# HybridRobotics/ilqr-iterative-tasks

Hardware: AMD Instinct MI355X
Metric: batched iLQR iterations/s (n=6,m=2,N=20) (higher is better)
Workload: dtype f64

## Files before the change

### ilqr_iterative_tasks_amd/csrc/i2lqr_group.hip

```cpp
#include "i2lqr_group.h"

#include "i2lqr_devcfg.hpp"
#include "i2lqr_geometry.hpp"
#include "i2lqr_group.hpp"
#include "i2lqr_dryrun.hpp"

namespace i2lqr {

namespace {

template <class T, class Sys, int G = kGroup> size_t group_lds_bytes(int N) {
  return (size_t)GLayout<Sys, G>(N).wave_words() * sizeof(T);
}

bool has_stage_weights(const i2lqr_config& cfg) {
  for (int i = 0; i < cfg.n; i++)
    for (int j = 0; j < cfg.n; j++)
      if (cfg.Q[i * I2LQR_MAX_N + j] != 0.0) return true;
  for (int a = 0; a < cfg.m; a++)
    for (int b = 0; b < cfg.m; b++)
      if (cfg.R[a * I2LQR_MAX_M + b] != 0.0) return true;
  return false;
}

template <auto Kernel> hipError_t raise_lds_limit(size_t lds) {
  if (lds <= device_geometry().default_dyn_lds) return hipSuccess;
  constexpr int kMaxDev = 64;
  static thread_local int raised_for[kMaxDev] = {};
  int dev = 0;
  hipError_t e = hipGetDevice(&dev);
  if (e != hipSuccess) return e;
  if (dev < 0 || dev >= kMaxDev || raised_for[dev] < (int)lds) {
    e = hipFuncSetAttribute((const void*)Kernel, hipFuncAttributeMaxDynamicSharedMemorySize,
                            (int)lds);
    if (e != hipSuccess) return e;
    if (dev >= 0 && dev < kMaxDev) raised_for[dev] = (int)lds;
  }
  return hipSuccess;
}

template <class T, class Sys, int H, int G = kGroup>
hipError_t launch_h(const i2lqr_config& cfg, const IterArgs<T>& a, hipStream_t s) {
  const auto c = make_dev_cfg<T, Sys::n, Sys::m>(cfg);
  const size_t lds = group_lds_bytes<T, Sys, G>(cfg.N);
  if (hipError_t e = raise_lds_limit<k_group_iterate<T, Sys, H, false, G>>(lds); e != hipSuccess)
    return e;
  constexpr int PW = 64 / G;
  const unsigned grid = (unsigned)((a.B + PW - 1) / PW);
  hipLaunchKernelGGL((k_group_iterate<T, Sys, H, false, G>), dim3(grid), dim3(64 * H), lds, s, c, a,
                     (T*)nullptr);
  return hipGetLastError();
}
template <class T, class Sys>
hipError_t launch16(const i2lqr_config& cfg, const IterArgs<T>& a, hipStream_t s) {
  const int64_t cus = device_geometry().cus;
#ifndef I2LQR_STAMPS
  if ((a.B + 3) / 4 <= 2 * cus) return launch_h<T, Sys, 2, 16>(cfg, a, s);
#endif
  return launch_h<T, Sys, 1, 16>(cfg, a, s);
}
template <class T, class Sys>
hipError_t launch_ws(const i2lqr_config& cfg, const IterArgs<T>& a, void* ws, hipStream_t s) {
  const auto c = make_dev_cfg<T, Sys::n, Sys::m>(cfg);
  const size_t lds = (size_t)GLayout<Sys>(cfg.N, true).wave_words() * sizeof(T);
  if (hipError_t e = raise_lds_limit<k_group_iterate<T, Sys, 1, true>>(lds); e != hipSuccess) return e;
  const unsigned grid = (unsigned)((a.B + kGroupsPerWave - 1) / kGroupsPerWave);
  hipLaunchKernelGGL((k_group_iterate<T, Sys, 1, true>), dim3(grid), dim3(64), lds, s, c, a, (T*)ws);
  return hipGetLastError();
}

template <class T, class Sys>
hipError_t launch(const i2lqr_config& cfg, const IterArgs<T>& a, hipStream_t s) {
  const int64_t cus = device_geometry().cus;
#ifndef I2LQR_STAMPS
  if ((a.B + kGroupsPerWave - 1) / kGroupsPerWave <= cus) return launch_h<T, Sys, 3>(cfg, a, s);
#endif
  return launch_h<T, Sys, 1>(cfg, a, s);
}

constexpr int kSpecWideBatch = 512;

template <class T, class Sys, int V, int G = kGroup> size_t spec_lds_bytes(int N) {
  return (size_t)GSpecLayout<Sys, V, G>(N).group_words() * sizeof(T);
}

template <class T, class Sys, int V, bool SETIO, int G>
hipError_t launch_spec_v(const i2lqr_config& cfg, const IterArgs<T>& a, hipStream_t s) {
  const auto c = make_dev_cfg<T, Sys::n, Sys::m>(cfg);
  const size_t lds = spec_lds_bytes<T, Sys, V, G>(cfg.N);
  if (hipError_t e = raise_lds_limit<k_group_spec<T, Sys, V, SETIO, G>>(lds); e != hipSuccess)
    return e;
  constexpr int PW = 64 / G;
  const int64_t problems = SETIO ? (int64_t)a.count_max : a.B;
  const unsigned grid = (unsigned)((problems + PW - 1) / PW);
  hipLaunchKernelGGL((k_group_spec<T, Sys, V, SETIO, G>), dim3(grid), dim3(64 * V), lds, s, c, a);
  return hipGetLastError();
}
template <class T, class Sys, bool SETIO, int G>
hipError_t launch_spec(const i2lqr_config& cfg, const IterArgs<T>& a, hipStream_t s) {
  const DeviceGeometry& geo = device_geometry();
  const bool wide = !SETIO && a.B <= geo.scaled(kSpecWideBatch) &&
                    spec_lds_bytes<T, Sys, 3, G>(cfg.N) <= geo.max_dyn_lds;
  if (wide) return launch_spec_v<T, Sys, 3, SETIO, G>(cfg, a, s);
  return launch_spec_v<T, Sys, 2, SETIO, G>(cfg, a, s);
}
template <class T, bool SETIO>
hipError_t launch_spec_any(const i2lqr_config& cfg, const IterArgs<T>& a, hipStream_t s, int lanes) {
  const bool b4 = cfg.system_id == I2LQR_SYS_BICYCLE4;
  if (lanes == 16)
    return b4 ? launch_spec<T, Bicycle4<T>, SETIO, 16>(cfg, a, s)
              : launch_spec<T, Bicycle6<T>, SETIO, 16>(cfg, a, s);
  return b4 ? launch_spec<T, Bicycle4<T>, SETIO, kGroup>(cfg, a, s)
            : launch_spec<T, Bicycle6<T>, SETIO, kGroup>(cfg, a, s);
}

template <int G> bool spec_lds_fits(const i2lqr_config& cfg) {
  const size_t lds = cfg.dtype == I2LQR_F64
      ? (cfg.system_id == I2LQR_SYS_BICYCLE4 ? spec_lds_bytes<double, Bicycle4<double>, 2, G>(cfg.N)
                                             : spec_lds_bytes<double, Bicycle6<double>, 2, G>(cfg.N))
      : (cfg.system_id == I2LQR_SYS_BICYCLE4 ? spec_lds_bytes<float, Bicycle4<float>, 2, G>(cfg.N)
                                             : spec_lds_bytes<float, Bicycle6<float>, 2, G>(cfg.N));
  return lds <= device_geometry().max_dyn_lds;
}
bool spec_plant_ok(const i2lqr_config& cfg) {
  if (cfg.system_id != I2LQR_SYS_BICYCLE4 && cfg.system_id != I2LQR_SYS_BICYCLE6) return false;
  return !has_stage_weights(cfg);
}

}

bool group_spec_supported(const i2lqr_config& cfg, int lanes) {
  if (!spec_plant_ok(cfg) || cfg.layout != I2LQR_LAYOUT_PROBLEM_MAJOR) return false;
  return lanes == 16 ? spec_lds_fits<16>(cfg) : (group_supported(cfg) && spec_lds_fits<kGroup>(cfg));
}
int group_spec_tail_lanes(const i2lqr_config& cfg) {
  if (!spec_plant_ok(cfg)) return 0;
  return spec_lds_fits<16>(cfg) ? 16 : (spec_lds_fits<kGroup>(cfg) ? kGroup : 0);
}
bool group_spec_tail_supported(const i2lqr_config& cfg) { return group_spec_tail_lanes(cfg) != 0; }

template <class T, class Sys>
hipError_t launch_spec_chain(const i2lqr_config& cfg, const IterArgs<T>& a, hipStream_t s) {
  const auto c = make_dev_cfg<T, Sys::n, Sys::m>(cfg);
  const size_t lds = spec_lds_bytes<T, Sys, 3, 16>(cfg.N);
  if (hipError_t e = raise_lds_limit<k_group_spec<T, Sys, 3, false, 16, true>>(lds); e != hipSuccess)
    return e;
  const unsigned grid = (unsigned)((a.B + 3) / 4);
  hipLaunchKernelGGL((k_group_spec<T, Sys, 3, false, 16, true>), dim3(grid), dim3(64 * 3), lds, s, c, a);
  return hipGetLastError();
}
bool group_spec_chain_supported(const i2lqr_config& cfg, int64_t chains) {
  if (!spec_plant_ok(cfg) || cfg.layout != I2LQR_LAYOUT_PROBLEM_MAJOR) return false;
  const DeviceGeometry& geo = device_geometry();
  if (chains > geo.scaled(kSpecWideBatch)) return false;
  const size_t lds = cfg.dtype == I2LQR_F64
      ? (cfg.system_id == I2LQR_SYS_BICYCLE4 ? spec_lds_bytes<double, Bicycle4<double>, 3, 16>(cfg.N)
                                             : spec_lds_bytes<double, Bicycle6<double>, 3, 16>(cfg.N))
      : (cfg.system_id == I2LQR_SYS_BICYCLE4 ? spec_lds_bytes<float, Bicycle4<float>, 3, 16>(cfg.N)
// ... 103 lines not shown
```

### ilqr_iterative_tasks_amd/csrc/i2lqr_group.hpp

```cpp
#pragma once
#include <hip/hip_runtime.h>
#include <stdint.h>

#include "i2lqr_systems.hpp"
#include "i2lqr_wave.hpp"

namespace i2lqr {

constexpr int kGroup = 8;
constexpr int kGroupsPerWave = 64 / kGroup;

template <class Sys> struct GroupPattern {
  static constexpr int n = Sys::n, m = Sys::m, W = n + m, NV = Sys::NVAR;
  static constexpr int dt_row(int b) {
    for (int i = 2; i < n; i++)
      if (i != b && Sys::pat(i, b) == 2) return i;
    return -1;
  }
  static constexpr bool column_ok(int b) {
    int extra = 0;
    for (int i = 0; i < n; i++) {
      const int code = Sys::pat(i, b);
      if (i < 2) {
        if (code == 2) return false;
        if (i == b && code != 1) return false;
        continue;
      }
      if (i == b) {
        if (code != 1) return false;
      } else if (code == 2) {
        extra++;
      } else if (code != 0) {
        return false;
      }
    }
    return extra <= 1;
  }
  static constexpr bool ok() {
    if (W > kGroup || n + 1 > kGroup || n < 2) return false;
    for (int b = 0; b < W; b++)
      if (!column_ok(b)) return false;
    return true;
  }
};

#ifndef I2LQR_GROUP_UNROLL
#define I2LQR_GROUP_UNROLL 4
#endif
template <class Sys, int G = kGroup> struct GLayout {
  static constexpr int n = Sys::n, m = Sys::m, W = n + m, NV = Sys::NVAR, NT = Sys::NTRIG;
  static constexpr int PW = 64 / G;
  static constexpr int KW = (n + 1 + 1) & ~1;
  static constexpr int R_JV = 0, R_ZERO = NV, R_ONE = NV + 1, R_LU = NV + 2, R_LUU = NV + 2 + m,
                       R_OB = NV + 2 + 2 * m, RW = (NV + 2 + 2 * m + 5 + 1) & ~1;
  int N;
  static constexpr int kT1Stride = 80;
  int XU0, XU1, Kk, R, TR0, TR1, total;
  __host__ __device__ explicit GLayout(int N_, bool ws = false) : N(N_) {
    int o = 0;
    XU0 = o; o += W * (N + 1); o = (o + 3) & ~3;
    XU1 = o; o += W * (N + 1); o = (o + 3) & ~3;
    Kk = o; o += ws ? m * KW : m * KW * N; o = (o + 3) & ~3;
    R = o; o += ws ? 0 : RW * (N + 1);
    TR0 = o; o += NT * (N + 1); o = (o + 3) & ~3;
    TR1 = o; o += NT * (N + 1); o = (o + 3) & ~3;
    o = (o + 3) & ~3;
    if (((o / 4) & 1) == 0) o += 4;
    total = o;
  }
  __host__ __device__ int t1_base() const { return PW * total; }
  __host__ __device__ int qt_base() const { return t1_base() + (G == kGroup ? PW * kT1Stride : 0); }
  __host__ __device__ int ctl_base() const { return (qt_base() + n * n + 3) & ~3; }
  __host__ __device__ int wave_words() const { return ctl_base() + 16; }
  __host__ __device__ int ws_rec() const { return 0; }
  __host__ __device__ int ws_gain() const { return RW * (N + 1); }
  __host__ __device__ int ws_words() const { return (RW * (N + 1) + m * KW * N + 15) & ~15; }
};


template <int L> __device__ __forceinline__ void bcast_fmac1(double& a, double s, double c) {
  asm("v_fmac_f64_dpp %0, %1, %2 row_newbcast:%3 row_mask:0xf bank_mask:0xf" : "+v"(a) : "v"(s), "v"(c), "n"(L));
}
template <int L> __device__ __forceinline__ void bcast_fmac1(float& a, float s, float c) {
  asm("v_fmac_f32_dpp %0, %1, %2 row_newbcast:%3 row_mask:0xf bank_mask:0xf" : "+v"(a) : "v"(s), "v"(c), "n"(L));
}
template <int L, class T, int R>
__device__ __forceinline__ void bcast_fmac(T (&a)[R], const T (&s)[R], T c) {
#pragma unroll
  for (int r = 0; r < R; r++) bcast_fmac1<L>(a[r], s[r], c);
}
template <int L> __device__ __forceinline__ double bcast_mov(double v) {
  long long x = __builtin_bit_cast(long long, v);
  x = __builtin_amdgcn_mov_dpp(x, 0x150 + L, 0xf, 0xf, false);
  return __builtin_bit_cast(double, x);
}
template <int L> __device__ __forceinline__ float bcast_mov(float v) {
  int x = __builtin_bit_cast(int, v);
  x = __builtin_amdgcn_mov_dpp(x, 0x150 + L, 0xf, 0xf, false);
  return __builtin_bit_cast(float, x);
}
template <class T, int R> __device__ __forceinline__ void dpp_ready(T (&v)[R]) {
  if constexpr (R == 8)
    asm("s_nop 1" : "+v"(v[0]), "+v"(v[1]), "+v"(v[2]), "+v"(v[3]), "+v"(v[4]), "+v"(v[5]), "+v"(v[6]), "+v"(v[7]));
  else if constexpr (R == 6)
    asm("s_nop 1" : "+v"(v[0]), "+v"(v[1]), "+v"(v[2]), "+v"(v[3]), "+v"(v[4]), "+v"(v[5]));
  else static_assert(R == 6 || R == 8, "dpp_ready: n + m of the bicycles");
}

template <class T, class Sys, bool WS = false, int G = kGroup> struct GroupWorker {
  static constexpr int n = Sys::n, m = Sys::m, W = n + m, NV = Sys::NVAR, NT = Sys::NTRIG;
  static constexpr int NA = n + 1;
  using Cfg = DevCfg<T, n, m>;
  using GL = GLayout<Sys, G>;
  static_assert(G == kGroup || G == 16, "eight lanes per problem, or one 16-lane DPP row");
  static_assert(G == kGroup || !WS, "the workspace form is built for eight lanes per problem");
  using GP = GroupPattern<Sys>;
  static_assert(GP::ok(), "plant does not have the column structure this kernel is written for");
  const Cfg& c;
  const GL L;
  const Slice<T> S;
  const T* const Qt;
  const int g;
  const int N;
  int oR, oKk;
  T* T1c;
  int rho;
  T* Wp = nullptr;

  int off_c0, off_c1;
  int off_l0, off_l1;
  int off_lu[m];
  T own, cdt;
  int rsrc;
#ifdef I2LQR_STAMPS
  mutable unsigned long long st_acc[8] = {0, 0, 0, 0, 0, 0, 0, 0}, st_t0 = 0, st_t1 = 0;
#endif

  __device__ GroupWorker(const Cfg& c_, T* smem, int lane)
      : GroupWorker(c_, smem + (lane / G) * GL(c_.N, WS).total,
                    smem + GL(c_.N, WS).qt_base(), lane % G,
                    GL(c_.N, WS).total) {
    const int p = lane / G;
    if constexpr (G == kGroup) T1c = smem + L.t1_base() + p * GL::kT1Stride;
    rho = (p >> 1) & 1;
  }
  __device__ __forceinline__ T* rec(int t) const {
    if constexpr (WS) return Wp + L.ws_rec() + t * GL::RW;
    else return S + oR + t * GL::RW;
  }
  __device__ __forceinline__ T* gain(int t) const {
    if constexpr (WS) return Wp + L.ws_gain() + t * (m * GL::KW);
    else return S + oKk + t * (m * GL::KW);
  }
  __device__ __forceinline__ T* gain_x(int t) const {
    if constexpr (WS) return S + oKk;
    else return S + oKk + t * (m * GL::KW);
  }
  __device__ __forceinline__ void ws_publish() const {
    if constexpr (WS) {
      __builtin_amdgcn_fence(__ATOMIC_RELEASE, "workgroup");
      __builtin_amdgcn_s_waitcnt(0);
      wave_sync();
      __builtin_amdgcn_fence(__ATOMIC_ACQUIRE, "workgroup");
    }
  }
  __device__ __forceinline__ int t1_word(int col, int row) const {
    return (row >> 1) * (2 * kGroup) + ((col + rho) & (kGroup - 1)) * 2 + (row & 1);
  }

  __device__ GroupWorker(const Cfg& c_, T* slice, const T* qt, int g_, int slice_words)
      : c(c_), L(c_.N, WS), S(make_slice(slice, slice_words, c_.trap, TAG_GROUP_LDS)), Qt(qt),
        g(g_), N(c_.N) {
    oR = L.R; oKk = L.Kk;
    T1c = nullptr;
    rho = 0;
    off_c0 = GL::R_ZERO; off_c1 = GL::R_ZERO; off_l0 = GL::R_ZERO; off_l1 = GL::R_ZERO;
#pragma unroll
    for (int a = 0; a < m; a++) off_lu[a] = GL::R_ZERO;
    own = T(0); cdt = T(0); rsrc = 0;
    static_for_i<0, W>([&](auto b_) {
      constexpr int b = decltype(b_)::value;
      if (g == b && b < n) {
        constexpr int c0 = Sys::pat(0, b), c1 = Sys::pat(1, b);
        off_c0 = c0 == 0 ? GL::R_ZERO : (c0 == 1 ? GL::R_ONE : GL::R_JV + (c0 - 3));
        off_c1 = c1 == 0 ? GL::R_ZERO : (c1 == 1 ? GL::R_ONE : GL::R_JV + (c1 - 3));
        own = (b >= 2) ? T(1) : T(0);
        constexpr int r = GP::dt_row(b);
        cdt = r >= 0 ? c.dt : T(0);
        rsrc = r >= 0 ? r : 0;
        if (b < 2) {
          off_l0 = GL::R_OB + 2 + b;
          off_l1 = GL::R_OB + 3 + b;
        }
      }
    });
    if (g == n) {
      own = T(1);
      off_l0 = GL::R_OB + 0;
      off_l1 = GL::R_OB + 1;
#pragma unroll
      for (int a = 0; a < m; a++) off_lu[a] = GL::R_LU + a;
    }
    if constexpr (G == 16) {
      own = T(1);
      if (g == 0) off_c0 = GL::R_ZERO;
      if (g == 1) off_c1 = GL::R_ZERO;
    }
  }

  __device__ __forceinline__ T terminal_cost(const T (&x)[n], const T (&xT)[n]) const {
    T d[n];
#pragma unroll
    for (int i = 0; i < n; i++) d[i] = x[i] - xT[i];
    T acc = T(0);
#pragma unroll
    for (int j = 0; j < n; j++) {
      T col = T(0);
#pragma unroll
      for (int i = 0; i < n; i++) col += d[i] * Qt[i * n + j];
      acc += col * d[j];
    }
    return acc;
  }

  template <int i, int a> __device__ __forceinline__ void f_acc(T& acc, bool& first, T v,
                                                                const T (&jv)[NV]) const {
    constexpr int code = Sys::pat(i, a);
    if constexpr (code == 0) {
      return;
    } else if constexpr (code == 1) {
      acc = first ? v : acc + v;
      first = false;
    } else {
      const T f = code == 2 ? c.dt : jv[code >= 3 ? code - 3 : 0];
      acc = first ? f * v : t_fma(f, v, acc);
      first = false;
    }
  }

  __device__ __forceinline__ T rollout(int XUo, int TRo, const T (&xT)[n]) const {
    T x[n], u[m], xn[n], tr[NT];
#pragma unroll
    for (int i = 0; i < n; i++) x[i] = S[XUo + i];
    for (int t = 0; t < N; t++) {
#pragma unroll
      for (int a = 0; a < m; a++) u[a] = clip(S[XUo + t * W + n + a], -c.u_max[a], c.u_max[a]);
#pragma unroll
      for (int a = 0; a < m; a++) S[XUo + t * W + n + a] = u[a];
      Sys::trig(x, tr);
#pragma unroll
      for (int q = 0; q < NT; q++) S[TRo + t * NT + q] = tr[q];
      Sys::step_tr(c, x, u, tr, xn);
#pragma unroll
      for (int i = 0; i < n; i++) S[XUo + (t + 1) * W + i] = xn[i];
#pragma unroll
      for (int i = 0; i < n; i++) x[i] = xn[i];
    }
    Sys::trig(x, tr);
#pragma unroll
    for (int q = 0; q < NT; q++) S[TRo + N * NT + q] = tr[q];
    const T cost = terminal_cost(x, xT);
    wave_sync();
    return cost;
  }

  __device__ __forceinline__ void prep(int XUo, int TRo, const T (&ob)[6], T pa, T pb, int first,
                                       int stride) const {
    const bool has_ob = ob[5] >= T(0);
    const int opt = has_ob ? (int)ob[5] : 0;
    const T spd_y = opt == 1 ? ob[4] : T(0), spd_x = opt == 2 ? ob[4] : T(0);
    const int rounds = (N + stride) / stride;
    for (int r = 0; r < rounds; r++) {
      const int t0 = first + r * stride;
      const int t = t0 < N ? t0 : N;
      const int ts = t0 < N ? t0 : N - 1;
      T* Rs = rec(ts);
      {
        T xe[n], tr[NT], u[m], jv[NV];
#pragma unroll
        for (int i = 0; i < n; i++) xe[i] = S[XUo + (ts + 1) * W + i];
#pragma unroll
        for (int a = 0; a < m; a++) u[a] = S[XUo + ts * W + n + a];
#pragma unroll
        for (int q = 0; q < NT; q++) tr[q] = S[TRo + (ts + 1) * NT + q];
        Sys::jac_var(c, xe, u, tr, jv);
#pragma unroll
        for (int q = 0; q < NV; q++) Rs[GL::R_JV + q] = jv[q];
#pragma unroll
        for (int a = 0; a < m; a++) {
          T e_hi, e_lo;
          if (sizeof(T) == 8 && c.fast_barrier) {
            e_hi = t_exp_bounded(c.ctrl_q2 * (u[a] - c.u_max[a]));
            e_lo = c.ctrl_c[a] * t_rcp(e_hi);
          } else {
            e_hi = t_exp(c.ctrl_q2 * (u[a] - c.u_max[a]));
            e_lo = t_exp(c.ctrl_q2 * (-c.u_max[a] - u[a]));
          }
          Rs[GL::R_LU + a] = c.ctrl_q12 * e_hi - c.ctrl_q12 * e_lo;
          Rs[GL::R_LUU + a] = c.ctrl_q122 * e_hi +
                              c.ctrl_q122 * e_lo;
        }
      }
      T* R = rec(t);
      R[GL::R_ZERO] = T(0);
      R[GL::R_ONE] = T(1);
      const T px = S[XUo + t * W + 0], py = S[XUo + t * W + 1];
      const T dz = opt == 2 ? px - (ob[0] - T(t) * spd_x) : px - ob[0];
      const T dy = opt == 1 ? py - (ob[1] + T(t) * spd_y) : py - ob[1];
      const T h = T(1) + c.safety_margin - (dz * pa * dz + dy * pb * dy);
      const T hd0 = T(-2) * pa * dz, hd1 = T(-2) * pb * dy;
      const T e = t_exp(c.obs_q2 * h);
      const T c1 = c.obs_q12 * e, c2 = c.obs_q122 * e;
      R[GL::R_OB + 0] = has_ob ? c1 * hd0 : T(0);
      R[GL::R_OB + 1] = has_ob ? c1 * hd1 : T(0);
      R[GL::R_OB + 2] = has_ob ? c2 * (hd0 * hd0) : T(0);
      R[GL::R_OB + 3] = has_ob ? c2 * (hd0 * hd1) : T(0);
      R[GL::R_OB + 4] = has_ob ? c2 * (hd1 * hd1) : T(0);
    }
    wave_sync();
    ws_publish();
  }

  __device__ __forceinline__ void quu_inverse(const T (&Quu)[m * m], T lamb, T (&inv)[m * m]) const {
    static_assert(m == 2, "the eight-lane kernel is written for m == 2 plants");
    t_quu_inverse2(Quu, lamb, inv);
  }

  template <bool GENERAL>
  __device__ __forceinline__ bool backward(int XUo, const T (&xT)[n], T lamb, bool commit) const {
    if constexpr (G == 16) return backward_row<GENERAL>(XUo, xT, lamb, commit);
    bool bad = false;
    T va[n];
    {
      const T* Rn = rec(N);
      T dx[n];
#pragma unroll
      for (int i = 0; i < n; i++) dx[i] = S[XUo + N * W + i] - xT[i];
#pragma unroll
      for (int i = 0; i < n; i++) {
        T vxx = T(0), vx = T(0);
#pragma unroll
        for (int r = 0; r < n; r++) {
          const T q = T(2) * Qt[i * n + r];
          vxx = (g == r) ? q : vxx;
          vx += q * dx[r];
        }
        va[i] = (g == n) ? vx : vxx;
      }
      va[0] += Rn[off_l0];
      va[1] += Rn[off_l1];
    }
    const int gcol = g < GL::KW ? g : GL::KW - 1;
    struct Rec { T jv[NV], luu[m], c0, c1, l0, l1, lrow[m]; };
    Rec ra, rb;
    auto load_record = [&](int t, Rec& r) __attribute__((always_inline)) {
      const T* R = rec(t);
#pragma unroll
      for (int q = 0; q < NV; q++) r.jv[q] = R[GL::R_JV + q];
#pragma unroll
      for (int a = 0; a < m; a++) r.luu[a] = R[GL::R_LUU + a];
      r.c0 = R[off_c0];
      r.c1 = R[off_c1];
      r.l0 = R[off_l0];
      r.l1 = R[off_l1];
#pragma unroll
      for (int a = 0; a < m; a++) r.lrow[a] = R[off_lu[a]];
    };
    load_record(N - 1, ra);
    auto step = [&](const int t, Rec& rc, Rec& rn) __attribute__((always_inline)) {
      if constexpr (WS) load_record(t > 0 ? t - 1 : 0, rn);
      const T (&jv)[NV] = rc.jv;
      const T (&luu)[m] = rc.luu;
      const T (&lrow)[m] = rc.lrow;
      const T c0 = rc.c0, c1 = rc.c1, l0 = rc.l0, l1 = rc.l1;
      STAMP_BEGIN();
      T t1[W];
      static_for_i<0, W>([&](auto a_) {
        constexpr int a = decltype(a_)::value;
        T acc = T(0);
        bool first = true;
        static_for_i<0, n>([&](auto i_) {
          constexpr int i = decltype(i_)::value;
          f_acc<i, a>(acc, first, va[i], jv);
        });
        t1[a] = acc;
      });
#pragma unroll
      for (int a = 0; a < W; a++) T1c[t1_word(g, a)] = t1[a];
      wave_sync();
      STAMP_END(1);
      T h[W];
      {
        T s0[W], s1[W], sr[W];
#pragma unroll
        for (int a = 0; a < W; a++) {
          s0[a] = T1c[t1_word(0, a)];
          s1[a] = T1c[t1_word(1, a)];
          sr[a] = T1c[t1_word(rsrc, a)];
        }
#pragma unroll
        for (int a = 0; a < W; a++) {
          T acc = c0 * s0[a];
          acc = t_fma(c1, s1[a], acc);
          acc = t_fma(own, t1[a], acc);
          acc = t_fma(cdt, sr[a], acc);
          h[a] = acc;
        }
        h[0] += l0;
        h[1] += l1;
#pragma unroll
        for (int a = 0; a < m; a++) h[n + a] += lrow[a];
      }
      STAMP_END(2);
      T Quu[m * m], Qinv[m * m];
      static_for_i<0, m>([&](auto a_) {
        constexpr int a = decltype(a_)::value;
        static_for_i<0, m>([&](auto b_) {
          constexpr int b = decltype(b_)::value;
          T acc = T(0);
          bool first = true;
          static_for_i<0, n>([&](auto i_) {
            constexpr int i = decltype(i_)::value;
            if constexpr (Sys::pat(i, n + b) != 0) f_acc<i, n + b>(acc, first, T1c[t1_word(i, n + a)], jv);
          });
          Quu[a * m + b] = (a == b ? luu[a] : T(0)) + acc;
        });
      });
      if constexpr (GENERAL) quu_inverse(Quu, lamb, Qinv);
      else t_quu_inverse2_pd(Quu, lamb, Qinv, &bad);
      STAMP_END(3);
      T kc[m];
#pragma unroll
      for (int a = 0; a < m; a++) {
        T acc = T(0);
#pragma unroll
        for (int b = 0; b < m; b++) acc = t_fma(Qinv[a * m + b], h[n + b], acc);
        kc[a] = -acc;
      }
      T* Kt = gain_x(t);
      if constexpr (WS) {
        T* Kg = gain(t);
#pragma unroll
        for (int a = 0; a < m; a++) {
          Kt[a * GL::KW + gcol] = kc[a];
          if (commit) Kg[a * GL::KW + gcol] = kc[a];
        }
      } else {
#pragma unroll
        for (int a = 0; a < m; a++)
          if (commit) Kt[a * GL::KW + gcol] = kc[a];
      }
      wave_sync();
      STAMP_END(4);
      T kr[m][n];
#pragma unroll
      for (int a = 0; a < m; a++)
#pragma unroll
        for (int i = 0; i < n; i++) kr[a][i] = Kt[a * GL::KW + i];
      if constexpr (!WS) load_record(t > 0 ? t - 1 : 0, rn);
      T qk[m];
#pragma unroll
      for (int a = 0; a < m; a++) {
        T acc = T(0);
#pragma unroll
        for (int b = 0; b < m; b++) acc = t_fma(Quu[a * m + b], kc[b], acc);
        qk[a] = acc;
      }
#pragma unroll
      for (int i = 0; i < n; i++) {
        T acc = T(0);
#pragma unroll
        for (int a = 0; a < m; a++) acc = t_fma(kr[a][i], qk[a], acc);
        va[i] = h[i] - acc;
      }
      STAMP_END(5);
    };
    int t = N - 1;
    if constexpr (I2LQR_GROUP_UNROLL >= 4) {
      for (; t >= 3; t -= 4) {
        step(t, ra, rb);
        step(t - 1, rb, ra);
        step(t - 2, ra, rb);
        step(t - 3, rb, ra);
      }
    }
    for (; t >= 1; t -= 2) {
      step(t, ra, rb);
      step(t - 1, rb, ra);
    }
    if (t == 0) step(0, ra, rb);
    ws_publish();
    return bad;
  }

  template <bool GENERAL>
  __device__ __forceinline__ bool backward_row(int XUo, const T (&xT)[n], T lamb, bool commit) const {
    static_assert(GL::KW > n + 1, "the padding word of a gain row takes the stores of idle lanes");
    bool bad = false;
    T va[n];
    {
      const T* Rn = rec(N);
      T dx[n];
#pragma unroll
      for (int i = 0; i < n; i++) dx[i] = S[XUo + N * W + i] - xT[i];
      const int gq = g < n ? g : 0;
#pragma unroll
      for (int i = 0; i < n; i++) {
        T vx = T(0);
#pragma unroll
        for (int r = 0; r < n; r++) vx += (T(2) * Qt[i * n + r]) * dx[r];
        const T vxx = T(2) * Qt[i * n + gq];
        va[i] = (g == n) ? vx : (g < n ? vxx : T(0));
      }
      va[0] += Rn[off_l0];
      va[1] += Rn[off_l1];
    }
    const int gcol = (commit && g <= n) ? g : GL::KW - 1;
    T cdr[n];
#pragma unroll
    for (int r = 0; r < n; r++) cdr[r] = (rsrc == r) ? cdt : T(0);
    struct Rec { T jv[NV], luu[m], c0, c1, l0, l1, lrow[m]; };
    Rec ra, rb;
    auto load_record = [&](int t, Rec& r) __attribute__((always_inline)) {
      const T* R = rec(t);
#pragma unroll
      for (int q = 0; q < NV; q++) r.jv[q] = R[GL::R_JV + q];
#pragma unroll
      for (int a = 0; a < m; a++) r.luu[a] = R[GL::R_LUU + a];
      r.c0 = R[off_c0];
      r.c1 = R[off_c1];
      r.l0 = R[off_l0];
      r.l1 = R[off_l1];
#pragma unroll
      for (int a = 0; a < m; a++) r.lrow[a] = R[off_lu[a]];
    };
    auto f_entry = [&](auto k_, auto b_, const T (&jv)[NV]) __attribute__((always_inline)) {
      constexpr int code = Sys::pat(decltype(k_)::value, n + decltype(b_)::value);
      if constexpr (code == 1) return T(1);
      else if constexpr (code == 2) return c.dt;
      else return jv[code >= 3 ? code - 3 : 0];
    };
    load_record(N - 1, ra);
    auto step = [&](const int t, Rec& rc, Rec& rn) __attribute__((always_inline)) {
      const T (&jv)[NV] = rc.jv;
      T t1[W];
      static_for_i<0, W>([&](auto a_) {
        constexpr int a = decltype(a_)::value;
        T acc = T(0);
        bool first = true;
        static_for_i<0, n>([&](auto i_) {
          constexpr int i = decltype(i_)::value;
          f_acc<i, a>(acc, first, va[i], jv);
        });
        t1[a] = acc;
      });
      dpp_ready(t1);
      load_record(t > 0 ? t - 1 : 0, rn);
      T Quu[m * m], Qinv[m * m];
      {
        T t1u[m];
#pragma unroll
        for (int a = 0; a < m; a++) t1u[a] = t1[n + a];
        static_for_i<0, m>([&](auto b_) {
          constexpr int b = decltype(b_)::value;
          T col[m];
#pragma unroll
          for (int a = 0; a < m; a++) col[a] = (a == b) ? rc.luu[a] : T(0);
          static_for_i<0, n>([&](auto k_) {
            constexpr int k = decltype(k_)::value;
            if constexpr (Sys::pat(k, n + b) != 0) bcast_fmac<k>(col, t1u, f_entry(k_, b_, jv));
          });
#pragma unroll
          for (int a = 0; a < m; a++) Quu[a * m + b] = col[a];
        });
      }
      auto h_rows = [&](auto r0_, auto& hr) __attribute__((always_inline)) {
        constexpr int r0 = decltype(r0_)::value;
        constexpr int R = sizeof(hr) / sizeof(T);
        T src[R];
#pragma unroll
        for (int a = 0; a < R; a++) { src[a] = t1[r0 + a]; hr[a] = t1[r0 + a]; }
        bcast_fmac<0>(hr, src, rc.c0);
        bcast_fmac<1>(hr, src, rc.c1);
        static_for_i<2, n>([&](auto r_) {
          constexpr int r = decltype(r_)::value;
          constexpr bool used = [] {
            for (int b = 0; b < n; b++)
              if (GP::dt_row(b) == r) return true;
            return false;
          }();
          if constexpr (used) bcast_fmac<r>(hr, src, cdr[r]);
        });
      };
      T hu[m], hx[n];
      h_rows(std::integral_constant<int, n>{}, hu);
#pragma unroll
      for (int a = 0; a < m; a++) hu[a] += rc.lrow[a];
      if constexpr (GENERAL) quu_inverse(Quu, lamb, Qinv);
      else t_quu_inverse2_pd(Quu, lamb, Qinv, &bad);
      h_rows(std::integral_constant<int, 0>{}, hx);
      hx[0] += rc.l0;
      hx[1] += rc.l1;
      T pk[m], kc[m];
#pragma unroll
      for (int a = 0; a < m; a++) {
        T acc = T(0);
#pragma unroll
        for (int b = 0; b < m; b++) acc = t_fma(Qinv[a * m + b], hu[b], acc);
        pk[a] = acc;
        kc[a] = -acc;
      }
      T* Kt = gain_x(t);
#pragma unroll
      for (int a = 0; a < m; a++) Kt[a * GL::KW + gcol] = kc[a];
      T qk[m];
#pragma unroll
      for (int a = 0; a < m; a++) {
        T acc = T(0);
#pragma unroll
        for (int b = 0; b < m; b++) acc = t_fma(Quu[a * m + b], kc[b], acc);
        qk[a] = acc;
      }
      T vn[n];
#pragma unroll
      for (int i = 0; i < n; i++) vn[i] = hx[i];
      static_for_i<0, n>([&](auto i_) {
        constexpr int i = decltype(i_)::value;
#pragma unroll
        for (int a = 0; a < m; a++) bcast_fmac1<i>(vn[i], pk[a], qk[a]);
      });
#pragma unroll
      for (int i = 0; i < n; i++) va[i] = vn[i];
    };
    STAMP_BEGIN();
    int t = N - 1;
    if constexpr (I2LQR_GROUP_UNROLL >= 4) {
      for (; t >= 3; t -= 4) {
        step(t, ra, rb);
        step(t - 1, rb, ra);
        step(t - 2, ra, rb);
        step(t - 3, rb, ra);
      }
    }
    for (; t >= 1; t -= 2) {
      step(t, ra, rb);
      step(t - 1, rb, ra);
    }
    if (t == 0) step(0, ra, rb);
    STAMP_END(1);
    wave_sync();
    return bad;
  }

  __device__ __forceinline__ T forward_row(int XUo, int XUn, int TRn, const T (&xT)[n],
                                           bool* bad) const {
    static_assert(G == 16 && m == 2, "two inputs on the two halves of a 16-lane row");
    const int half = g >> 3;
    const T umax = half ? c.u_max[1] : c.u_max[0];
    T x[n], u[m], xn[n], tr[NT];
#pragma unroll
    for (int i = 0; i < n; i++) x[i] = S[XUo + i];
#pragma unroll
    for (int i = 0; i < n; i++) S[XUn + i] = x[i];
    Sys::template trig_g<false>(x, tr, bad);
#pragma unroll
    for (int q = 0; q < NT; q++) S[TRn + q] = tr[q];
    static_assert(!WS, "gain rows and records are neighbours in the LDS slice");
    auto pXo = S + XUo;
    auto pXn = S + XUn;
    auto pG = S + (oKk + half * GL::KW);
    auto pTR = S + (TRn + half * NT);
    T xo[n], uo, kk[NA];
    auto load_step = [&](auto k_) __attribute__((always_inline)) {
      constexpr int k = decltype(k_)::value;
#pragma unroll
      for (int j = 0; j < n; j++) xo[j] = pXo[k * W + j];
      uo = pXo[k * W + n + half];
#pragma unroll
      for (int j = 0; j < NA; j++) kk[j] = pG[k * (m * GL::KW) + j];
    };
    load_step(std::integral_constant<int, 0>{});
    auto step = [&](auto k_, const T (&trc)[NT]) __attribute__((always_inline)) {
      constexpr int k = decltype(k_)::value;
      T acc = T(0);
#pragma unroll
      for (int j = 0; j < n; j++) acc = t_fma(kk[j], x[j] - xo[j], acc);
      const T ua = clip(uo + kk[n] + acc, -umax, umax);
      load_step(std::integral_constant<int, k + 1>{});
      pXn[k * W + n + half] = ua;
      u[0] = bcast_mov<0>(ua);
      u[1] = bcast_mov<8>(ua);
      Sys::step_tr(c, x, u, trc, xn);
#pragma unroll
      for (int i = 0; i < n; i++) pXn[(k + 1) * W + i] = xn[i];
#pragma unroll
      for (int i = 0; i < n; i++) x[i] = xn[i];
    };
    int t = 0;
    for (; t + 1 < N; t += 2) {
      step(std::integral_constant<int, 0>{}, tr);
      T sc[NT], tr1[NT];
      Sys::trig_heading_fast(half ? Sys::next_heading(c, x) : Sys::heading(x), sc, bad);
#pragma unroll
      for (int q = 0; q < NT; q++) pTR[NT + q] = sc[q];
#pragma unroll
      for (int q = 0; q < NT; q++) {
        tr1[q] = bcast_mov<0>(sc[q]);
        tr[q] = bcast_mov<8>(sc[q]);
      }
      step(std::integral_constant<int, 1>{}, tr1);
      pXo = pXo + 2 * W;
      pXn = pXn + 2 * W;
      pG = pG + 2 * (m * GL::KW);
      pTR = pTR + 2 * NT;
    }
    if (t < N) {
      step(std::integral_constant<int, 0>{}, tr);
      Sys::template trig_g<false>(x, tr, bad);
#pragma unroll
      for (int q = 0; q < NT; q++) S[TRn + N * NT + q] = tr[q];
    }
    const T cost = terminal_cost(x, xT);
    wave_sync();
    return cost;
  }

  template <bool GENERAL>
  __device__ __forceinline__ T forward(int XUo, int XUn, int TRn, const T (&xT)[n],
                                       bool* bad) const {
    if constexpr (G == 16 && !GENERAL && Sys::kHeadingAhead && m == 2)
      return forward_row(XUo, XUn, TRn, xT, bad);
    T x[n], u[m], xn[n], tr[NT];
#pragma unroll
    for (int i = 0; i < n; i++) x[i] = S[XUo + i];
#pragma unroll
    for (int i = 0; i < n; i++) S[XUn + i] = x[i];
    T xo[n], uo[m];
    struct Gains { T kk[m][NA]; };
    Gains ga, gb;
    auto load_gains = [&](int t, Gains& q) __attribute__((always_inline)) {
      const T* Kg = gain(t);
#pragma unroll
      for (int a = 0; a < m; a++)
#pragma unroll
        for (int j = 0; j < NA; j++) q.kk[a][j] = Kg[a * GL::KW + j];
    };
    auto load_step = [&](int t, Gains& q) __attribute__((always_inline)) {
#pragma unroll
      for (int j = 0; j < n; j++) xo[j] = S[XUo + t * W + j];
#pragma unroll
      for (int a = 0; a < m; a++) uo[a] = S[XUo + t * W + n + a];
      if constexpr (!WS) load_gains(t, q);
    };
    if constexpr (WS) {
      load_gains(0, ga);
      load_gains(N >= 2 ? 1 : 0, gb);
    }
    load_step(0, ga);
    auto step = [&](const int t, Gains& q, Gains& qn) __attribute__((always_inline)) {
#pragma unroll
      for (int a = 0; a < m; a++) {
        T acc = T(0);
#pragma unroll
        for (int j = 0; j < n; j++) acc = t_fma(q.kk[a][j], x[j] - xo[j], acc);
        u[a] = clip(uo[a] + q.kk[a][n] + acc, -c.u_max[a], c.u_max[a]);
      }
      if constexpr (WS) {
        load_gains(t + 2 < N ? t + 2 : N - 1, q);
        load_step(t + 1 < N ? t + 1 : t, qn);
      } else {
        load_step(t + 1 < N ? t + 1 : t, q);
      }
#pragma unroll
      for (int a = 0; a < m; a++) S[XUn + t * W + n + a] = u[a];
      Sys::template trig_g<GENERAL>(x, tr, bad);
#pragma unroll
      for (int q = 0; q < NT; q++) S[TRn + t * NT + q] = tr[q];
      Sys::step_tr(c, x, u, tr, xn);
#pragma unroll
      for (int i = 0; i < n; i++) S[XUn + (t + 1) * W + i] = xn[i];
#pragma unroll
      for (int i = 0; i < n; i++) x[i] = xn[i];
    };
    int t = 0;
    if constexpr (WS) {
      for (; t + 1 < N; t += 2) {
        step(t, ga, gb);
        step(t + 1, gb, ga);
      }
      if (t < N) step(t, ga, gb);
    } else {
      if constexpr (I2LQR_GROUP_UNROLL >= 4) {
        for (; t + 3 < N; t += 4) {
          step(t, ga, ga);
          step(t + 1, ga, ga);
          step(t + 2, ga, ga);
          step(t + 3, ga, ga);
        }
      }
      for (; t + 1 < N; t += 2) {
        step(t, ga, ga);
        step(t + 1, ga, ga);
      }
      if (t < N) step(t, ga, ga);
    }
    Sys::template trig_g<GENERAL>(x, tr, bad);
#pragma unroll
    for (int q = 0; q < NT; q++) S[TRn + N * NT + q] = tr[q];
    const T cost = terminal_cost(x, xT);
    wave_sync();
    return cost;
  }
};

__device__ __forceinline__ int idx_div(int e, int d, float rcp_d) {
  int q = (int)((float)e * rcp_d);
  const int r = e - q * d;
  q += (r >= d) ? 1 : 0;
  q -= (r < 0) ? 1 : 0;
  return q;
}

template <class T, class Sys, int H = 1, bool WS = false, int G = kGroup>
__global__ __launch_bounds__(64 * H) void k_group_iterate(const DevCfg<T, Sys::n, Sys::m> c,
                                                          const IterArgs<T> a, T* ws = nullptr) {
  static_assert(!(WS && H > 1), "the workspace form runs without helper wavefronts");
  constexpr int n = Sys::n, m = Sys::m, W = n + m;
  using GL = GLayout<Sys, G>;
  extern __shared__ __align__(16) unsigned char gsmem_raw[];
  T* smem = reinterpret_cast<T*>(gsmem_raw);
  const int lane = threadIdx.x & 63, hv = threadIdx.x >> 6;
#ifdef I2LQR_STAMPS
  unsigned long long st_k0, st_k1, st_k2, st_k3;
  asm volatile("s_memtime %0\n\ts_waitcnt lgkmcnt(0)" : "=s"(st_k0)::"memory");
#endif
  const int64_t prob0 = (int64_t)blockIdx.x * GL::PW + lane / G;
  const bool real = prob0 < a.B;
  const int64_t prob = real ? prob0 : a.B - 1;
  GroupWorker<T, Sys, WS, G> w(c, smem, lane);
  const int N = c.N, g = w.g;
  const float rN = 1.0f / (float)N, rN1 = 1.0f / (float)(N + 1), rnN = 1.0f / (float)(n * N);
  const GL& L = w.L;
  const auto S = w.S;
  if constexpr (WS) w.Wp = ws + prob0 * (int64_t)L.ws_words();

  if (H == 1 || hv == 0) {
    const T* gX = a.X + prob * (int64_t)(n * (N + 1));
    if (g < n) S[L.XU0 + g] = gX[g * (N + 1)];
    const T* gU = a.U + prob * (int64_t)(m * N);
    for (int e = g; e < m * N; e += G) {
      const int aa = idx_div(e, N, rN), t = e - aa * N;
      S[L.XU0 + t * W + n + aa] = gU[e];
    }
    for (int e = lane; e < n * n; e += 64) smem[L.qt_base() + e] = c.Qt[e];
  }
  T xT[n], ob[6];
#pragma unroll
  for (int i = 0; i < n; i++) xT[i] = a.x_term[prob * n + i];
#pragma unroll
  for (int q = 0; q < 6; q++) ob[q] = a.obs ? a.obs[prob * 6 + q] : T(q == 5 ? -1 : 1);
  T lamb = a.lamb[prob];
  wave_sync();

  int cur = 0;
  const T ob_pa = T(1) / (ob[2] * ob[2]), ob_pb = T(1) / (ob[3] * ob[3]);
  int* const ctl = reinterpret_cast<int*>(smem + L.ctl_base());
  if constexpr (H > 1) {
    if (hv > 0) {
      for (;;) {
        __syncthreads();
        const int flags = ctl[8];
        if (!(flags & 1)) break;
        if (flags & 2) {
          const int pc = ctl[lane / G];
          w.prep(pc ? L.XU1 : L.XU0, pc ? L.TR1 : L.TR0, ob, ob_pa, ob_pb, hv * G + g,
                 H * G);
        }
        __syncthreads();
      }
      return;
    }
  }
  T cost = w.rollout(L.XU0, L.TR0, xT);
  int it = 0, status = a.early_exit ? 2  : 0 ;
  T cost_ret = cost;
  bool fresh = true, active = a.n_iters > 0;
#ifdef I2LQR_STAMPS
  asm volatile("s_memtime %0\n\ts_waitcnt lgkmcnt(0)" : "=s"(st_k1)::"memory");
#endif
  while (__any(active)) {
    const int XUo = cur ? L.XU1 : L.XU0, XUn = cur ? L.XU0 : L.XU1;
    const int TRo = cur ? L.TR1 : L.TR0, TRn = cur ? L.TR0 : L.TR1;
#ifdef I2LQR_STAMPS
    {
      auto& st_t0 = w.st_t0; auto& st_t1 = w.st_t1; auto& st_acc = w.st_acc;
      STAMP_BEGIN();
      if (__any(fresh)) w.prep(XUo, TRo, ob, ob_pa, ob_pb, g, G);
      STAMP_END(0);
    }
#else
    if constexpr (H > 1) {
      const bool do_prep = __any(fresh);
      if (g == 0) ctl[lane / G] = cur;
      if (lane == 0) ctl[8] = 1 | (do_prep ? 2 : 0);
      __syncthreads();
      if (do_prep) w.prep(XUo, TRo, ob, ob_pa, ob_pb, g, H * G);
      __syncthreads();
    } else {
      if (__any(fresh)) w.prep(XUo, TRo, ob, ob_pa, ob_pb, g, G);
    }
#endif
    if (__builtin_expect(__any(w.template backward<false>(XUo, xT, lamb, active)), 0))
      w.template backward<true>(XUo, xT, lamb, active);
    T cost_new;
    {
#ifdef I2LQR_STAMPS
      auto& st_t0 = w.st_t0; auto& st_t1 = w.st_t1; auto& st_acc = w.st_acc;
      STAMP_BEGIN();
#endif
      bool big = false;
      cost_new = w.template forward<false>(XUo, XUn, TRn, xT, &big);
      if (__builtin_expect(__any(big), 0)) cost_new = w.template forward<true>(XUo, XUn, TRn, xT, &big);
#ifdef I2LQR_STAMPS
      STAMP_END(6);
#endif
    }
    {
      const bool acc = active && cost_new < cost, rej = active && !(cost_new < cost);
      const T lamb_dn = lamb / c.lamb_factor, lamb_up = lamb * c.lamb_factor;
      const bool conv = t_abs((cost_new - cost) / cost) < c.eps;
      it += active ? 1 : 0;
      fresh = acc;
      cur ^= acc ? 1 : 0;
      lamb = acc ? lamb_dn : (rej ? lamb_up : lamb);
      cost_ret = acc ? cost_new : (rej ? cost : cost_ret);
      cost = acc ? cost_new : cost;
      const bool stop_conv = acc && conv, stop_lamb = rej && lamb > c.max_lamb;
      const int ended = stop_conv ? 1 : 3;
      if (a.early_exit) {
        status = (stop_conv || stop_lamb) ? ended : status;
        active = active && !(stop_conv || stop_lamb);
      } else {
        status = (status == 0 && (stop_conv || stop_lamb)) ? ended : status;
      }
      active = active && it < a.n_iters;
    }
  }
#ifdef I2LQR_STAMPS
  asm volatile("s_memtime %0\n\ts_waitcnt lgkmcnt(0)" : "=s"(st_k2)::"memory");
#endif
  if constexpr (H > 1) {
    if (lane == 0) ctl[8] = 0;
    __syncthreads();
  }
  if (!t_isfinite(cost_ret)) status = 4;

  if (real) {
    const int XUo = cur ? L.XU1 : L.XU0;
    T* gX = a.X + prob * (int64_t)(n * (N + 1));
    for (int e = g; e < n * (N + 1); e += G) {
      const int i = idx_div(e, N + 1, rN1), t = e - i * (N + 1);
      gX[e] = S[XUo + t * W + i];
    }
    T* gU = a.U + prob * (int64_t)(m * N);
    for (int e = g; e < m * N; e += G) {
      const int aa = idx_div(e, N, rN), t = e - aa * N;
      gU[e] = S[XUo + t * W + n + aa];
    }
    if (a.K) {
      T* gK = a.K + prob * (int64_t)(m * n * N);
      for (int e = g; e < m * n * N; e += G) {
        const int aa = idx_div(e, n * N, rnN), r = e - aa * (n * N);
        const int j = idx_div(r, N, rN), t = r - j * N;
        gK[e] = w.gain(t)[aa * GL::KW + j];
      }
      T* gk = a.k + prob * (int64_t)(m * N);
      for (int e = g; e < m * N; e += G) {
        const int aa = idx_div(e, N, rN), t = e - aa * N;
        gk[e] = w.gain(t)[aa * GL::KW + n];
      }
    }
    if (g == 0) {
      a.lamb[prob] = lamb;
      a.cost[prob] = cost_ret;
      if (a.iters) a.iters[prob] = it;
      if (a.status) a.status[prob] = status;
    }
#ifdef I2LQR_STAMPS
    asm volatile("s_waitcnt vmcnt(0)\n\ts_memtime %0\n\ts_waitcnt lgkmcnt(0)" : "=s"(st_k3)::"memory");
    w.st_acc[2] = st_k1 - st_k0;
    w.st_acc[3] = st_k2 - st_k1;
    w.st_acc[4] = st_k3 - st_k2;
    if (a.dbg && g == 0)
      for (int q = 0; q < 8; q++) a.dbg[prob * 8 + q] = w.st_acc[q];
#endif
  }
  if (a.qfun) {
    const bool cand = real && g == 0;
    T ci = T(0);
    if (cand) {
      const int XUo = cur ? L.XU1 : L.XU0;
      double ss = 0.0;
#pragma unroll
      for (int i = 0; i < n; i++) {
        const double d = (double)S[XUo + N * W + i] - (double)xT[i];
        ss += d * d;
      }
      ci = (T)relax_cost_value(ss, a.qfun[prob], N, a.outer_iter, a.max_relax_iter);
// ... 243 lines not shown
```

Before: 70.96 million.

## Pipeline helper-wave record prep with the forward pass using double-buffered records

In multi-wave (H>1) launches, helper waves now build the stage records for the candidate trajectory while the main wave runs its forward pass. They work in eight-step chunks synchronised through hooks in the forward loop, and results go into a second record buffer, so prep is taken off the critical path between iterations. Records are double-buffered per problem, which needs extra LDS, and the H>1 paths are only chosen when that fits. The cost is many more block barriers per iteration, plus speculative prep work that is thrown away on rejected steps.

```diff
diff --git a/ilqr_iterative_tasks_amd/csrc/i2lqr_group.hip b/ilqr_iterative_tasks_amd/csrc/i2lqr_group.hip
--- a/ilqr_iterative_tasks_amd/csrc/i2lqr_group.hip
+++ b/ilqr_iterative_tasks_amd/csrc/i2lqr_group.hip
@@ -11,6 +11,9 @@
 
 template <class T, class Sys, int G = kGroup> size_t group_lds_bytes(int N) {
   return (size_t)GLayout<Sys, G>(N).wave_words() * sizeof(T);
+}
+template <class T, class Sys, int G = kGroup> size_t group_lds_bytes_h(int N) {
+  return (size_t)GLayout<Sys, G>(N).wave_words_h() * sizeof(T);
 }
 
 bool has_stage_weights(const i2lqr_config& cfg) {
@@ -42,7 +45,7 @@
 template <class T, class Sys, int H, int G = kGroup>
 hipError_t launch_h(const i2lqr_config& cfg, const IterArgs<T>& a, hipStream_t s) {
   const auto c = make_dev_cfg<T, Sys::n, Sys::m>(cfg);
-  const size_t lds = group_lds_bytes<T, Sys, G>(cfg.N);
+  const size_t lds = H > 1 ? group_lds_bytes_h<T, Sys, G>(cfg.N) : group_lds_bytes<T, Sys, G>(cfg.N);
   if (hipError_t e = raise_lds_limit<k_group_iterate<T, Sys, H, false, G>>(lds); e != hipSuccess)
     return e;
   constexpr int PW = 64 / G;
@@ -53,10 +56,9 @@
 }
 template <class T, class Sys>
 hipError_t launch16(const i2lqr_config& cfg, const IterArgs<T>& a, hipStream_t s) {
-  const int64_t cus = device_geometry().cus;
-#ifndef I2LQR_STAMPS
-  if ((a.B + 3) / 4 <= 2 * cus) return launch_h<T, Sys, 2, 16>(cfg, a, s);
-#endif
+  const DeviceGeometry& geo = device_geometry();
+  if ((a.B + 3) / 4 <= 2 * geo.cus && group_lds_bytes_h<T, Sys, 16>(cfg.N) <= geo.max_dyn_lds)
+    return launch_h<T, Sys, 2, 16>(cfg, a, s);
   return launch_h<T, Sys, 1, 16>(cfg, a, s);
 }
 template <class T, class Sys>
@@ -73,7 +75,9 @@
 hipError_t launch(const i2lqr_config& cfg, const IterArgs<T>& a, hipStream_t s) {
   const int64_t cus = device_geometry().cus;
 #ifndef I2LQR_STAMPS
-  if ((a.B + kGroupsPerWave - 1) / kGroupsPerWave <= cus) return launch_h<T, Sys, 3>(cfg, a, s);
+  if ((a.B + kGroupsPerWave - 1) / kGroupsPerWave <= cus &&
+      group_lds_bytes_h<T, Sys>(cfg.N) <= device_geometry().max_dyn_lds)
+    return launch_h<T, Sys, 3>(cfg, a, s);
 #endif
   return launch_h<T, Sys, 1>(cfg, a, s);
 }
diff --git a/ilqr_iterative_tasks_amd/csrc/i2lqr_group.hpp b/ilqr_iterative_tasks_amd/csrc/i2lqr_group.hpp
--- a/ilqr_iterative_tasks_amd/csrc/i2lqr_group.hpp
+++ b/ilqr_iterative_tasks_amd/csrc/i2lqr_group.hpp
@@ -72,6 +72,12 @@
   __host__ __device__ int qt_base() const { return t1_base() + (G == kGroup ? PW * kT1Stride : 0); }
   __host__ __device__ int ctl_base() const { return (qt_base() + n * n + 3) & ~3; }
   __host__ __device__ int wave_words() const { return ctl_base() + 16; }
+  __host__ __device__ int rec2_stride() const {
+    const int o = (RW * (N + 1) + 3) & ~3;
+    return ((o / 4) & 1) ? o : o + 4;
+  }
+  __host__ __device__ int rec2_base() const { return wave_words(); }
+  __host__ __device__ int wave_words_h() const { return rec2_base() + PW * rec2_stride(); }
   __host__ __device__ int ws_rec() const { return 0; }
   __host__ __device__ int ws_gain() const { return RW * (N + 1); }
   __host__ __device__ int ws_words() const { return (RW * (N + 1) + m * KW * N + 15) & ~15; }
@@ -107,6 +113,10 @@
   else static_assert(R == 6 || R == 8, "dpp_ready: n + m of the bicycles");
 }
 
+struct NoHook {
+  __device__ __forceinline__ void operator()() const {}
+};
+
 template <class T, class Sys, bool WS = false, int G = kGroup> struct GroupWorker {
   static constexpr int n = Sys::n, m = Sys::m, W = n + m, NV = Sys::NVAR, NT = Sys::NTRIG;
   static constexpr int NA = n + 1;
@@ -266,14 +276,20 @@
 
   __device__ __forceinline__ void prep(int XUo, int TRo, const T (&ob)[6], T pa, T pb, int first,
                                        int stride) const {
+    prep_span(XUo, TRo, ob, pa, pb, 0, N + 1, first, stride);
+    wave_sync();
+    ws_publish();
+  }
+  __device__ __forceinline__ void prep_span(int XUo, int TRo, const T (&ob)[6], T pa, T pb, int lo,
+                                            int hi, int first, int stride) const {
     const bool has_ob = ob[5] >= T(0);
     const int opt = has_ob ? (int)ob[5] : 0;
     const T spd_y = opt == 1 ? ob[4] : T(0), spd_x = opt == 2 ? ob[4] : T(0);
-    const int rounds = (N + stride) / stride;
+    const int rounds = (hi - lo + stride - 1) / stride;
     for (int r = 0; r < rounds; r++) {
-      const int t0 = first + r * stride;
-      const int t = t0 < N ? t0 : N;
-      const int ts = t0 < N ? t0 : N - 1;
+      const int t0 = lo + first + r * stride;
+      const int t = t0 < hi ? t0 : hi - 1;
+      const int ts = t < N ? t : N - 1;
       T* Rs = rec(ts);
       {
         T xe[n], tr[NT], u[m], jv[NV];
@@ -317,8 +333,6 @@
       R[GL::R_OB + 3] = has_ob ? c2 * (hd0 * hd1) : T(0);
       R[GL::R_OB + 4] = has_ob ? c2 * (hd1 * hd1) : T(0);
     }
-    wave_sync();
-    ws_publish();
   }
 
   __device__ __forceinline__ void quu_inverse(const T (&Quu)[m * m], T lamb, T (&inv)[m * m]) const {
@@ -326,9 +340,10 @@
     t_quu_inverse2(Quu, lamb, inv);
   }
 
-  template <bool GENERAL>
-  __device__ __forceinline__ bool backward(int XUo, const T (&xT)[n], T lamb, bool commit) const {
-    if constexpr (G == 16) return backward_row<GENERAL>(XUo, xT, lamb, commit);
+  template <bool GENERAL, class Hook = NoHook>
+  __device__ __forceinline__ bool backward(int XUo, const T (&xT)[n], T lamb, bool commit,
+                                           Hook records_ready = {}) const {
+    if constexpr (G == 16) return backward_row<GENERAL>(XUo, xT, lamb, commit, records_ready);
     bool bad = false;
     T va[n];
     {
@@ -347,6 +362,7 @@
         }
         va[i] = (g == n) ? vx : vxx;
       }
+      records_ready();
       va[0] += Rn[off_l0];
       va[1] += Rn[off_l1];
     }
@@ -493,8 +509,9 @@
     return bad;
   }
 
-  template <bool GENERAL>
-  __device__ __forceinline__ bool backward_row(int XUo, const T (&xT)[n], T lamb, bool commit) const {
+  template <bool GENERAL, class Hook = NoHook>
+  __device__ __forceinline__ bool backward_row(int XUo, const T (&xT)[n], T lamb, bool commit,
+                                               Hook records_ready = {}) const {
     static_assert(GL::KW > n + 1, "the padding word of a gain row takes the stores of idle lanes");
     bool bad = false;
     T va[n];
@@ -512,6 +529,7 @@
         const T vxx = T(2) * Qt[i * n + gq];
         va[i] = (g == n) ? vx : (g < n ? vxx : T(0));
       }
+      records_ready();
       va[0] += Rn[off_l0];
       va[1] += Rn[off_l1];
     }
@@ -652,8 +670,9 @@
     return bad;
   }
 
+  template <class Hook = NoHook>
   __device__ __forceinline__ T forward_row(int XUo, int XUn, int TRn, const T (&xT)[n],
-                                           bool* bad) const {
+                                           bool* bad, Hook stored8 = {}) const {
     static_assert(G == 16 && m == 2, "two inputs on the two halves of a 16-lane row");
     const int half = g >> 3;
     const T umax = half ? c.u_max[1] : c.u_max[0];
@@ -696,8 +715,7 @@
 #pragma unroll
       for (int i = 0; i < n; i++) x[i] = xn[i];
     };
-    int t = 0;
-    for (; t + 1 < N; t += 2) {
+    auto pair = [&]() __attribute__((always_inline)) {
       step(std::integral_constant<int, 0>{}, tr);
       T sc[NT], tr1[NT];
       Sys::trig_heading_fast(half ? Sys::next_heading(c, x) : Sys::heading(x), sc, bad);
@@ -713,7 +731,16 @@
       pXn = pXn + 2 * W;
       pG = pG + 2 * (m * GL::KW);
       pTR = pTR + 2 * NT;
-    }
+    };
+    int t = 0;
+    for (; t + 7 < N; t += 8) {
+      pair();
+      pair();
+      pair();
+      pair();
+      stored8();
+    }
+    for (; t + 1 < N; t += 2) pair();
     if (t < N) {
       step(std::integral_constant<int, 0>{}, tr);
       Sys::template trig_g<false>(x, tr, bad);
@@ -725,11 +752,11 @@
     return cost;
   }
 
-  template <bool GENERAL>
+  template <bool GENERAL, class Hook = NoHook>
   __device__ __forceinline__ T forward(int XUo, int XUn, int TRn, const T (&xT)[n],
-                                       bool* bad) const {
+                                       bool* bad, Hook stored8 = {}) const {
     if constexpr (G == 16 && !GENERAL && Sys::kHeadingAhead && m == 2)
-      return forward_row(XUo, XUn, TRn, xT, bad);
+      return forward_row(XUo, XUn, TRn, xT, bad, stored8);
     T x[n], u[m], xn[n], tr[NT];
 #pragma unroll
     for (int i = 0; i < n; i++) x[i] = S[XUo + i];
@@ -796,6 +823,8 @@
           step(t + 1, ga, ga);
           step(t + 2, ga, ga);
           step(t + 3, ga, ga);
+          if constexpr (!std::is_same_v<Hook, NoHook>)
+            if ((t & 4) != 0) stored8();
         }
       }
       for (; t + 1 < N; t += 2) {
@@ -865,65 +894,92 @@
   int cur = 0;
   const T ob_pa = T(1) / (ob[2] * ob[2]), ob_pb = T(1) / (ob[3] * ob[3]);
   int* const ctl = reinterpret_cast<int*>(smem + L.ctl_base());
+  const int p = lane / G;
+  const int oR1 = H > 1 ? L.rec2_base() + p * L.rec2_stride() - p * L.total : L.R;
+  auto rec_of = [&](int b) { return b ? oR1 : L.R; };
+  static_assert(H == 1 || I2LQR_GROUP_UNROLL >= 4, "the forward pass's hook runs every eight steps");
+  const int n8 = N / 8;
   if constexpr (H > 1) {
     if (hv > 0) {
+      const int hg = (hv - 1) * G + g, hs = (H - 1) * G;
+      __syncthreads();
+      w.prep_span(L.XU0, L.TR0, ob, ob_pa, ob_pb, 0, N + 1, G + hg, H * G);
       for (;;) {
         __syncthreads();
-        const int flags = ctl[8];
-        if (!(flags & 1)) break;
-        if (flags & 2) {
-          const int pc = ctl[lane / G];
-          w.prep(pc ? L.XU1 : L.XU0, pc ? L.TR1 : L.TR0, ob, ob_pa, ob_pb, hv * G + g,
-                 H * G);
+        if (!(ctl[8] & 1)) break;
+        const int pc = ctl[p] ^ 1;
+        const int XUc = pc ? L.XU1 : L.XU0, TRc = pc ? L.TR1 : L.TR0;
+        w.oR = rec_of(pc);
+        int lo = 0;
+        for (int k = 0; k < n8; k++) {
+          __syncthreads();
+          const int hi = 8 * k + 7;
+          w.prep_span(XUc, TRc, ob, ob_pa, ob_pb, lo, hi, hg, hs);
+          lo = hi;
         }
         __syncthreads();
+        if (ctl[9]) {
+          __syncthreads();
+          lo = 0;
+        }
+        w.prep_span(XUc, TRc, ob, ob_pa, ob_pb, lo, N + 1, hg, hs);
       }
       return;
     }
   }
   T cost = w.rollout(L.XU0, L.TR0, xT);
+  if constexpr (H > 1) {
+    __syncthreads();
+    w.prep_span(L.XU0, L.TR0, ob, ob_pa, ob_pb, 0, N + 1, g, H * G);
+  }
   int it = 0, status = a.early_exit ? 2  : 0 ;
   T cost_ret = cost;
   bool fresh = true, active = a.n_iters > 0;
 #ifdef I2LQR_STAMPS
   asm volatile("s_memtime %0\n\ts_waitcnt lgkmcnt(0)" : "=s"(st_k1)::"memory");
+  auto& st_t0 = w.st_t0; auto& st_t1 = w.st_t1; auto& st_acc = w.st_acc;
 #endif
+  auto records_ready = [&]() __attribute__((always_inline)) {
+    STAMP_BEGIN();
+    __syncthreads();
+    STAMP_END(0);
+  };
+  auto stored8 = [&]() __attribute__((always_inline)) { __syncthreads(); };
   while (__any(active)) {
     const int XUo = cur ? L.XU1 : L.XU0, XUn = cur ? L.XU0 : L.XU1;
-    const int TRo = cur ? L.TR1 : L.TR0, TRn = cur ? L.TR0 : L.TR1;
-#ifdef I2LQR_STAMPS
-    {
-      auto& st_t0 = w.st_t0; auto& st_t1 = w.st_t1; auto& st_acc = w.st_acc;
+    const int TRn = cur ? L.TR0 : L.TR1;
+    w.oR = rec_of(cur);
+    if constexpr (H > 1) {
+      if (g == 0) ctl[p] = cur;
+      if (lane == 0) ctl[8] = 1;
+    } else {
+      const int TRo = cur ? L.TR1 : L.TR0;
       STAMP_BEGIN();
       if (__any(fresh)) w.prep(XUo, TRo, ob, ob_pa, ob_pb, g, G);
       STAMP_END(0);
     }
-#else
-    if constexpr (H > 1) {
-      const bool do_prep = __any(fresh);
-      if (g == 0) ctl[lane / G] = cur;
-      if (lane == 0) ctl[8] = 1 | (do_prep ? 2 : 0);
-      __syncthreads();
-      if (do_prep) w.prep(XUo, TRo, ob, ob_pa, ob_pb, g, H * G);
-      __syncthreads();
-    } else {
-      if (__any(fresh)) w.prep(XUo, TRo, ob, ob_pa, ob_pb, g, G);
-    }
-#endif
-    if (__builtin_expect(__any(w.template backward<false>(XUo, xT, lamb, active)), 0))
-      w.template backward<true>(XUo, xT, lamb, active);
+    bool bad_bw;
+    if constexpr (H > 1) bad_bw = __any(w.template backward<false>(XUo, xT, lamb, active, records_ready));
+    else bad_bw = __any(w.template backward<false>(XUo, xT, lamb, active));
+    if (__builtin_expect(bad_bw, 0)) w.template backward<true>(XUo, xT, lamb, active);
     T cost_new;
     {
-#ifdef I2LQR_STAMPS
-      auto& st_t0 = w.st_t0; auto& st_t1 = w.st_t1; auto& st_acc = w.st_acc;
       STAMP_BEGIN();
-#endif
       bool big = false;
-      cost_new = w.template forward<false>(XUo, XUn, TRn, xT, &big);
-      if (__builtin_expect(__any(big), 0)) cost_new = w.template forward<true>(XUo, XUn, TRn, xT, &big);
-#ifdef I2LQR_STAMPS
+      if constexpr (H > 1) {
+        cost_new = w.template forward<false>(XUo, XUn, TRn, xT, &big, stored8);
+        const bool redo = __any(big);
+        if (lane == 0) ctl[9] = redo ? 1 : 0;
+        __syncthreads();
+        if (__builtin_expect(redo, 0)) {
+          cost_new = w.template forward<true>(XUo, XUn, TRn, xT, &big);
+          __syncthreads();
+        }
+      } else {
+        cost_new = w.template forward<false>(XUo, XUn, TRn, xT, &big);
+        if (__builtin_expect(__any(big), 0)) cost_new = w.template forward<true>(XUo, XUn, TRn, xT, &big);
+      }
       STAMP_END(6);
-#endif
     }
     {
       const bool acc = active && cost_new < cost, rej = active && !(cost_new < cost);
```

Result: faster. 72.51 million, median of 6 (+2.2%).
